# smajida/openHEVC

Measured on AMD Instinct MI355X. Metric: decoded Mpixels/s (luma), synthetic stream, higher is better.
Workload: dtype u16

## Files before the change

openhevc_amd/csrc/engine_handover.hip:

```cpp
#include <memory>

#include "engine_impl.h"

hipEvent_t sync_event_get(OhEngine *e)
{
    hipEvent_t ev = nullptr;
    if (!e->sync_events.empty()) { ev = e->sync_events.back(); e->sync_events.pop_back(); return ev; }
    return hipEventCreateWithFlags(&ev, hipEventDisableTiming) == hipSuccess ? ev : nullptr;
}
void sync_event_put(OhEngine *e, hipEvent_t ev)
{
    if (!ev) return;
    if (e->sync_events.size() < 4096) e->sync_events.push_back(ev); else (void)hipEventDestroy(ev);
}

static void *arena_new(OhEngine *e, size_t bytes)
{
    void *p = nullptr;
    if (hipMalloc(&p, bytes) != hipSuccess)
        return nullptr;
    e->arenas_alive++; e->arena_bytes_alive += bytes;
    return p;
}
static void arena_delete(OhEngine *e, void *p, size_t bytes)
{
    (void)hipFree(p);
    if (e) { e->arenas_alive--; e->arena_bytes_alive -= bytes; }
}

static int arena_take(OhEngine *e, size_t total, OhChunk *ck)
{
    int best = -1;
    for (size_t i = 0; i < e->arenas.size() && best < 0; i++)
        if (e->arenas[i].bytes >= total && e->arenas[i].bytes <= 2 * total + (1u << 20))
            best = (int)i;
    if (best >= 0 && e->arenas[best].free_ev && hipEventQuery(e->arenas[best].free_ev) != hipSuccess && e->arenas.size() < 512)
        best = -1;
    if (best >= 0) {
        ck->arena = e->arenas[best].p; ck->arena_bytes = e->arenas[best].bytes;
        if (e->arenas[best].free_ev) {
            (void)hipStreamWaitEvent(e->copy_stream, e->arenas[best].free_ev, 0);
            sync_event_put(e, e->arenas[best].free_ev);
        }
        e->arenas.erase(e->arenas.begin() + best);
        return OH_OK;
    }
    ck->arena_bytes = align_up(total, (size_t)1 << 20);
    if ((ck->arena = arena_new(e, ck->arena_bytes)) == nullptr) {
        (void)hipStreamSynchronize(e->stream);
        for (auto &a : e->arenas) { sync_event_put(e, a.free_ev); arena_delete(e, a.p, a.bytes); }
        e->arenas.clear();
        if ((ck->arena = arena_new(e, ck->arena_bytes)) == nullptr)
            FAIL(e, OH_E_NOMEM, "hipMalloc(%zu) for the work lists failed", total);
    }
    return OH_OK;
}

static void chunk_free(OhEngine *e, OhChunk *ck, bool in_flight)
{
    if (e && ck->ready)
        sync_event_put(e, ck->ready);
    if (ck->sum_host) {
        if (e && e->sum_pool.size() < 4096) e->sum_pool.push_back(ck->sum_host);
        else (void)hipHostFree(ck->sum_host);
    }
    if (ck->arena) {
        if (e && e->arenas.size() < 1024) {
            hipEvent_t fe = nullptr;
            if (in_flight && (fe = sync_event_get(e)) != nullptr && hipEventRecord(fe, e->stream) != hipSuccess) {
                sync_event_put(e, fe);
                fe = nullptr;
            }
            if (in_flight && !fe)
                (void)hipStreamSynchronize(e->stream);
            e->arenas.push_back({ ck->arena, ck->arena_bytes, fe });
        } else {
            if (in_flight && e) (void)hipStreamSynchronize(e->stream);
            arena_delete(e, ck->arena, ck->arena_bytes);
        }
    }
    delete ck;
}

void free_dev_frame(OhEngine *e, OhDevFrame *df, bool in_flight)
{
    if (!df)
        return;
    OhChunk *ck = df->chunk;
    delete df;
    if (!ck)
        return;
    ck->in_flight = ck->in_flight || in_flight;
    if (--ck->refs <= 0)
        chunk_free(e, ck, ck->in_flight);
}

static bool same_geometry(const OhPicParams &a, const OhPicParams &b)
{
    return a.width == b.width && a.height == b.height && a.bit_depth == b.bit_depth && a.chroma_format_idc == b.chroma_format_idc;
}

static int check_host_side(OhEngine *e, const OhFrame *f, const Pic *cur, HostSide *h, std::vector<uint32_t> &pu_off)
{
    const OhPicParams &p = f->p;
    h->ref_ok = 0; h->ref_used = 0; h->n_cross = 0; h->any_dense = false;
    for (int i = 0; i < OH_MAX_REFS; i++) {
        Pic *r = get_pic(e, f->ref_pics[i]);
        if (r && same_geometry(r->p, p) && r != cur)
            h->ref_ok |= 1u << i;
    }
    if ((f->n_pu && !f->pu) || (f->n_wp && !f->wp) || (f->n_tu && !f->tu) || (f->n_intra && !f->intra))
        FAIL(e, OH_E_ARG, "a non-zero item count comes with a NULL array (pu / wp / tu / intra)");
    uint64_t nl = 0, nc = 0;
    const int hs = oh_hshift(&p, 1), vs = oh_vshift(&p, 1), two = p.chroma_format_idc ? 2 : 0;
    if ((uint64_t)f->n_pu * 2048 >= (1ull << 31))
        FAIL(e, OH_E_ARG, "PU list too long");
    pu_off.resize(2 * ((size_t)f->n_pu + 1));
    uint32_t *ol = pu_off.data(), *oc = ol + f->n_pu + 1;
    h->pu_off = ol;
    for (uint32_t i = 0; i < f->n_pu; i++) {
        const OhPu &pu = f->pu[i];
        ol[i] = (uint32_t)nl; oc[i] = (uint32_t)nc;
        nl += (uint64_t)(((pu.w + 7) >> 3) * ((pu.h + 7) >> 3));
        nc += (uint64_t)(two * ((((pu.w >> hs) + 7) >> 3) * (((pu.h >> vs) + 7) >> 3)));
        for (int l = 0; l < 2; l++)
            if (pu.ref[l] < OH_MAX_REFS) h->ref_used |= (uint16_t)(1u << pu.ref[l]);
    }
    ol[f->n_pu] = (uint32_t)nl; oc[f->n_pu] = (uint32_t)nc;
    for (uint32_t i = 0; i < f->n_wp; i++)
        if (f->wp[i].log2_denom[0] > 7 || f->wp[i].log2_denom[1] > 7)
            FAIL(e, OH_E_ARG, "weights %u: log2 denominator out of range", i);
    h->tu_cnt[0] = h->tu_cnt[1] = h->tu_cnt[2] = h->tu_cnt[3] = 0;
    for (uint32_t i = 0; i < f->n_tu; i++) {
        const OhTu &t = f->tu[i];
        h->tu_cnt[(t.log2_size - 2) & 3]++;
        h->n_cross += (t.flags & OH_TUF_CROSS) != 0;
        h->any_dense = h->any_dense || !(t.flags & OH_TUF_SPARSE);
    }
    if (h->any_dense && f->n_coeff && !f->coeffs)
        FAIL(e, OH_E_ARG, "dense transform blocks but coeffs[] is NULL");
    if (h->n_cross && !f->tu_cross)
        FAIL(e, OH_E_ARG, "cross-component blocks without tu_cross[]");
    if (f->n_intra && p.constrained_intra_pred && !f->is_intra)
        FAIL(e, OH_E_ARG, "constrained_intra_pred without the is_intra map");
    if (f->n_intra) {
        if (!f->level_start || !f->n_levels || !f->ictu || !f->n_ictu || !f->sub_start || !f->n_sub ||
            f->level_start[0] != 0 || f->level_start[f->n_levels] != f->n_ictu)
            FAIL(e, OH_E_ARG, "intra wavefront tables inconsistent");
        for (uint32_t l = 0; l < f->n_levels; l++)
            if (f->level_start[l] > f->level_start[l + 1])
                FAIL(e, OH_E_ARG, "intra level table not monotonic");
    }
    if (p.deblock_enabled) {
        const OhBsInputs *bi = f->bs_in;
        if (bi && (!bi->mvf || !bi->cbf_luma || !bi->call_log2 || !bi->ctb_flags))
            FAIL(e, OH_E_ARG, "bs_in: all four maps are required");
        if (bi && (p.log2_min_pu_size < 2 || p.log2_min_tb_size < 2))
            FAIL(e, OH_E_ARG, "bs_in: min PU / TB size below 4");
        if (bi) {
            const size_t n_cells = (size_t)(p.width >> p.log2_min_tb_size) * (p.height >> p.log2_min_tb_size);
            for (size_t i = 0; i < n_cells; i++)
                if (bi->call_log2[i] && (bi->call_log2[i] < p.log2_min_tb_size || bi->call_log2[i] > p.log2_ctb_size))
                    FAIL(e, OH_E_ARG, "bs_in: call_log2[%zu] = %d is not a block size of this picture", i, bi->call_log2[i]);
        }
        if ((!bi && (!f->vertical_bs || !f->horizontal_bs || f->bs_size < oh_bs_size(&p))) || !f->qp_y_tab || !f->deblock)
            FAIL(e, OH_E_ARG, "deblock side arrays missing or too small");
    }
    if ((p.pcm_loop_filter_disable || p.transquant_bypass_enable) && !f->is_pcm)
        FAIL(e, OH_E_ARG, "is_pcm map required when pcm loop-filter disable / transquant bypass is on");
    OhPrepCounts *cnt = &h->cnt;
    cnt->n_pu = f->n_pu; cnt->n_mc_luma = (uint32_t)nl; cnt->n_mc_chroma = (uint32_t)nc; cnt->n_tu = f->n_tu;
    cnt->n_intra = f->n_intra; cnt->n_sub = f->n_intra ? f->n_sub : 0; cnt->n_ictu = f->n_intra ? f->n_ictu : 0;
    return OH_OK;
}

static void *summary_block_get(OhEngine *e)
{
    void *p = nullptr;
    if (!e->sum_pool.empty()) { p = e->sum_pool.back(); e->sum_pool.pop_back(); return p; }
    return hipHostMalloc(&p, OH_MAX_BATCH * sizeof(DevSummary), hipHostMallocDefault) == hipSuccess ? p : nullptr;
}

static void fill_header(OhEngine *e, const OhFrame *f, const Pic *cur, const HostSide &h, const HandoverLayout &L, char *copied_base, char *rest_base,
                        OhDevFrame *df, HandoverHeader *H)
{
    DevFrame &hd = H->d;
    hd.pp = f->p;
    fill_planes(&hd.cur, cur, false);
    fill_planes(&hd.out, cur, f->p.sao_enabled && f->sao);
    for (int i = 0; i < OH_MAX_REFS; i++) {
        Pic *r = get_pic(e, f->ref_pics[i]);
        df->ref_id[i] = -1; df->ref_gen[i] = 0; df->ref_half[i] = 0;
        if (h.ref_ok >> i & 1) {
            fill_planes(&hd.refs[i], r, r->final_b);
            df->ref_id[i] = f->ref_pics[i]; df->ref_gen[i] = r->gen; df->ref_half[i] = r->final_b ? 1 : 0;
        }
    }
    df->ref_used = h.ref_used;
    df->cur_gen = cur->gen;
    handover_bind_split(L, copied_base, rest_base, H);
    hd.coeffs_present = f->coeffs != nullptr;
    hd.err_word = e->kerr; hd.cur_pic_id = f->cur_pic;
    hd.n_pu = f->n_pu; hd.n_mc_luma = h.cnt.n_mc_luma; hd.n_mc_chroma = h.cnt.n_mc_chroma; hd.n_tu = f->n_tu; hd.n_intra = f->n_intra;
    hd.n_ictu = h.cnt.n_ictu; hd.n_sub = h.cnt.n_sub; hd.n_levels = f->n_intra ? f->n_levels : 0; hd.n_wp = f->n_wp; hd.n_sparse = f->sparse ? f->n_sparse : 0;
    hd.ref_ok = h.ref_ok; hd.n_coeff = f->n_coeff;
    hd.n_cross = h.n_cross;
    for (int k = 0, first = 0; k < 4; k++) { hd.tu_first[k] = (uint32_t)first; hd.tu_cnt[k] = h.tu_cnt[k]; first += (int)h.tu_cnt[k]; }
    hd.dbg = e->dbg;
}

enum { PULL_TABLE = 64 };
static_assert(HL_N_SEGS <= PULL_TABLE, "a table entry per copied segment");
static size_t pulled_stage_bytes(const HandoverLayout &L) { return L.own_bytes + PULL_TABLE * sizeof(OhPullSeg); }
static hipError_t stage_pulled(OhEngine *e, const HandoverLayout &L, char *arena, OhEngine::Stage *sg)
{
    char *sp = (char *)sg->p;
    OhPullSeg *tab = (OhPullSeg *)(sp + L.own_bytes);
    int nt = 0;
    size_t pulled = 0;
    { HostTimer t(e, OH_HT_UPLOAD_MEMCPY);
    for (int i = 0; i < L.ns; i++)
        if (L.seg[i].own && L.seg[i].bytes) {
            memcpy(sp, L.seg[i].src, L.seg[i].bytes);
            tab[nt++] = OhPullSeg{ sp, arena + L.seg[i].off, L.seg[i].bytes };
            sp += align_up(L.seg[i].bytes, 256);
        }
    for (int i = 0; i < L.ns; i++)
        if (!L.seg[i].own && L.copied(L.seg[i])) {
            tab[nt++] = OhPullSeg{ L.seg[i].src, arena + L.seg[i].off, L.seg[i].bytes };
            pulled += L.seg[i].bytes;
        }
    }
    HostTimer t_enq(e, OH_HT_UPLOAD_ENQUEUE);
    ohk_pull(tab, nt, pulled, e->copy_stream);
    return hipGetLastError();
}

static hipError_t stage_copied(OhEngine *e, const HandoverLayout *L, const size_t *copied_off, int n, char *arena, size_t bytes, OhEngine::Stage *sg)
{
    { HostTimer t(e, OH_HT_UPLOAD_MEMCPY);
    if (!e->copiers) {
        static const char *cenv = getenv("OHEVC_COPY_THREADS");
        e->copiers = new CopyPool();
        e->copiers->start(cenv ? std::max(0, std::min(atoi(cenv), 8)) : 2);
    }
    e->copy_jobs.clear();
    for (int i = 0; i < n; i++)
        handover_copy_jobs_add(L[i], (char *)sg->p + (copied_off[i] - copied_off[0]), e->copy_jobs);
    e->copiers->run(e->copy_jobs);
    }
    HostTimer t_enq(e, OH_HT_UPLOAD_ENQUEUE);
    return hipMemcpyAsync(arena + copied_off[0], sg->p, bytes, hipMemcpyHostToDevice, e->copy_stream);
}

static hipError_t enqueue_bs_derive(const OhFrame *f, const HandoverHeader &H, hipStream_t cs)
{
    const size_t bs_packed = (oh_bs_size(&f->p) + 3) / 4;
    hipError_t hrc = hipMemsetAsync((void *)H.d.vbs, 0, align_up(bs_packed, 4), cs);
    if (hrc == hipSuccess) hrc = hipMemsetAsync((void *)H.d.hbs, 0, align_up(bs_packed, 4), cs);
    if (hrc == hipSuccess)
        ohk_bs_derive(&f->p, H.mvf, H.cbf_luma, H.call_log2, H.ctb_flags, f->bs_in->loop_filter_across_tiles, (void *)H.d.vbs, (void *)H.d.hbs, cs);
    return hrc;
}

struct ChunkScratch {
    HostSide h[OH_MAX_BATCH];
    std::vector<uint32_t> pu_off[OH_MAX_BATCH];
    HandoverHeader H[OH_MAX_BATCH];
    HandoverLayout L[OH_MAX_BATCH];
    Pic *cur[OH_MAX_BATCH];
};

static int upload_chunk(OhEngine *e, const OhFrame *const *fs, int n, OhDevFrame **out)
{
    static thread_local std::unique_ptr<ChunkScratch> scratch;
    if (!scratch) scratch.reset(new ChunkScratch());
    ChunkScratch &S = *scratch;
    HostTimer t_all(e, OH_HT_UPLOAD);
    for (int i = 0; i < n; i++) {
        const OhFrame *f = fs[i];
        if (!f)
            return OH_E_ARG;
        int rc = check_params(e, &f->p);
        if (rc)
            return rc;
        S.cur[i] = get_pic(e, f->cur_pic);
        if (!S.cur[i] || !same_geometry(S.cur[i]->p, f->p))
            FAIL(e, OH_E_ARG, "cur_pic %d is not an allocated picture of this geometry", f->cur_pic);
        { HostTimer t(e, OH_HT_UPLOAD_COUNT);
        rc = check_host_side(e, f, S.cur[i], &S.h[i], S.pu_off[i]);
        }
        if (rc)
            return rc;
        memset(&S.H[i], 0, sizeof(S.H[i]));
        S.L[i] = handover_layout(f, S.h[i], &S.H[i].d);
    }
    HIPCHK(e, hipSetDevice(e->device));
    const HandoverChunk C = handover_chunk_place(S.L, n);
    OhChunk *ck = new OhChunk();
    int rc;
    { HostTimer t(e, OH_HT_UPLOAD_ARENA);
    rc = arena_take(e, C.total, ck);
    }
    if (rc) {
        delete ck;
        return rc;
    }
    if ((ck->sum_host = summary_block_get(e)) == nullptr) {
        chunk_free(e, ck, false);
        FAIL(e, OH_E_NOMEM, "hipHostMalloc(%zu) for the summaries failed", OH_MAX_BATCH * sizeof(DevSummary));
    }
    char *arena = (char *)ck->arena;
    ck->refs = n;
    for (int i = 0; i < n; i++) {
        const OhFrame *f = fs[i];
        const HostSide &h = S.h[i];
        OhDevFrame *df = new OhDevFrame();
        df->chunk = ck;
        fill_header(e, f, S.cur[i], h, S.L[i], arena + C.copied_off[i], arena + C.rest_off[i], df, &S.H[i]);
        df->sum_host = (DevSummary *)ck->sum_host + i;
        S.H[i].d.summary_host = df->sum_host;
        df->sum_dev = S.H[i].d.summary;
        df->cnt = h.cnt;
        df->d = (DevFrame *)(arena + C.copied_off[i]);
        df->p = f->p;
        for (int k = 0; k < 4; k++) df->tu_cnt[k] = h.tu_cnt[k];
        df->n_cross = h.n_cross;
        df->has_sao = f->p.sao_enabled && f->sao;
        df->cur_pic = f->cur_pic;
        df->owner = e;
        out[i] = df;
    }

    hipStream_t cs = e->copy_stream;
    auto pulled = [&](int i) { return (fs[i]->flags & OH_FRAME_PINNED) != 0 && !S.L[i].packs; };
    for (int g0 = 0, g1; g0 < n; g0 = g1) {
        const bool pull = pulled(g0);
        for (g1 = g0 + 1; !pull && g1 < n && g1 - g0 < OH_STAGE_GROUP && !pulled(g1); g1++)
            ;
        const size_t bytes = C.copied_off[g1] - C.copied_off[g0];
        OhEngine::Stage *sg;
        { HostTimer t(e, OH_HT_UPLOAD_STAGE_WAIT);
        sg = stage_acquire(e, pull ? pulled_stage_bytes(S.L[g0]) : bytes);
        }
        if (!sg)
            FAIL(e, OH_E_NOMEM, "hipHostMalloc(%zu) failed", bytes);
        hipError_t hrc = pull ? stage_pulled(e, S.L[g0], arena + C.copied_off[g0], sg)
                              : stage_copied(e, &S.L[g0], &C.copied_off[g0], g1 - g0, arena, bytes, sg);
        HostTimer t_enq(e, OH_HT_UPLOAD_ENQUEUE);
        if (hrc == hipSuccess && stage_in_use(e, sg, cs) != OH_OK)
            hrc = hipGetLastError();
        for (int i = g0; i < g1; i++) {
            e->up_bytes += S.L[i].copy_bytes;
            if (hrc == hipSuccess && S.H[i].mvf)
                hrc = enqueue_bs_derive(fs[i], S.H[i], cs);
        }
        if (hrc != hipSuccess)
            FAIL(e, OH_E_HIP, "work-list upload failed: %s", hipGetErrorString(hrc));
    }

    HostTimer t_enq(e, OH_HT_UPLOAD_ENQUEUE);
    OhBatch B;
    memset(&B, 0, sizeof(B));
    OhPrepCounts mx;
    memset(&mx, 0, sizeof(mx));
    uint32_t max_cross = 0, max_runs = 0;
    for (int i = 0; i < n; i++) {
        const OhDevFrame *df = out[i];
        B.f[i] = df->d;
        mx.n_pu = std::max(mx.n_pu, df->cnt.n_pu); mx.n_tu = std::max(mx.n_tu, df->cnt.n_tu);
        mx.n_intra = std::max(mx.n_intra, df->cnt.n_intra); mx.n_sub = std::max(mx.n_sub, df->cnt.n_sub);
        mx.n_ictu = std::max(mx.n_ictu, df->cnt.n_ictu);
        max_runs = std::max(max_runs, ((df->cnt.n_mc_luma + 63) >> 6) + ((df->cnt.n_mc_chroma + 63) >> 6));
        max_cross = std::max(max_cross, df->n_cross);
    }
    ohk_prepare(&B, n, &mx, max_runs, max_cross, cs);
    HIPCHK(e, hipGetLastError());
    if ((ck->ready = sync_event_get(e)) == nullptr)
        FAIL(e, OH_E_NOMEM, "no event for the work lists");
    HIPCHK(e, hipEventRecord(ck->ready, cs));
    return OH_OK;
}

extern "C" int oh_frames_upload(OhEngine *e, const OhFrame *const *fs, int n, OhDevFrame **out)
{
    if (!e || n < 0 || (n && (!fs || !out)))
        return OH_E_ARG;
    for (int i = 0; i < n; i++) out[i] = nullptr;
    int rc = OH_OK;
    for (int c0 = 0; c0 < n && rc == OH_OK; c0 += OH_MAX_BATCH)
        rc = upload_chunk(e, fs + c0, n - c0 < OH_MAX_BATCH ? n - c0 : OH_MAX_BATCH, out + c0);
    if (rc != OH_OK) {
        bool any = false;
        for (int i = 0; i < n; i++) any = any || out[i];
        if (any) (void)hipStreamSynchronize(e->copy_stream);
        for (int i = 0; i < n; i++) { free_dev_frame(e, out[i]); out[i] = nullptr; }
    }
    return rc;
}

extern "C" int oh_frame_upload(OhEngine *e, const OhFrame *f, OhDevFrame **out)
{
    if (!e || !f || !out)
        return OH_E_ARG;
    return oh_frames_upload(e, &f, 1, out);
}
```

openhevc_amd/csrc/engine_impl.h:

```cpp
#ifndef OHEVC_ENGINE_IMPL_H
#define OHEVC_ENGINE_IMPL_H

#include <hip/hip_runtime.h>
#include <stdio.h>
#include <stdlib.h>
#include <string.h>
#include <algorithm>
#include <chrono>
#include <string>
#include <condition_variable>
#include <mutex>
#include <thread>
#include <vector>

#include "../../include/ohevc_hip.h"
#include "handover_layout.h"
#include "kernels.h"

#define OH_INTERNAL __attribute__((visibility("hidden")))

struct Pic {
    bool        used = false;
    OhPicParams p{};
    void       *base = nullptr;
    bool        owned = true;
    void       *a[3] = {}, *b[3] = {};
    int32_t     stride[3] = {}, w[3] = {}, h[3] = {};
    bool        final_b = false;
    uint32_t    gen = 0;
    uint64_t    done_seq = 0;
};

struct EventSet { hipEvent_t ev[OH_N_PASSES + 1]; int n_frames = 1; };

struct OhChunk {
    void      *arena = nullptr;
    size_t     arena_bytes = 0;
    hipEvent_t ready = nullptr;
    bool       waited = false;
    void      *sum_host = nullptr;
    int        refs = 0;
    bool       in_flight = false;
};

struct OhDevFrame {
    OhChunk   *chunk = nullptr;
    DevFrame  *d = nullptr;
    OhPicParams p{};
    uint32_t   tu_cnt[4] = { 0, 0, 0, 0 };
    uint32_t   n_cross = 0;
    bool       has_sao = false;
    int        cur_pic = -1;
    uint32_t   cur_gen = 0;
    int        ref_id[OH_MAX_REFS];
    uint32_t   ref_gen[OH_MAX_REFS];
    uint8_t    ref_half[OH_MAX_REFS];
    uint16_t   ref_used = 0;
    void      *sum_host = nullptr;
    bool       summary_read = false;
    void      *sum_dev = nullptr;
    OhPrepCounts cnt{};
    uint32_t   prep_err = 0;
    uint32_t   intra_area64 = 0, max_passes = 0;
    uint32_t   max_items = 0, max_sub = 0, max_res = 0;
    bool       res_scattered = false;
    uint64_t   sum_items = 0, sum_sub = 0;
    const struct OhEngine *owner = nullptr;
};

struct CopyPool {
    std::vector<std::thread> th;
    std::mutex mu;
    std::condition_variable cv, done_cv;
    const std::vector<CopyJob> *jobs = nullptr;
    int pending = 0;
    uint64_t gen = 0;
    bool stop = false;
    static void run_share(const std::vector<CopyJob> &jobs, int share, int shares)
    {
        for (size_t i = (size_t)share; i < jobs.size(); i += (size_t)shares) {
            const CopyJob &j = jobs[i];
            if (j.pack) pack_bs((uint8_t *)j.dst, (const uint8_t *)j.src, j.n);
            else memcpy(j.dst, j.src, j.n);
        }
    }
    void worker(int k)
    {
        uint64_t seen = 0;
        for (;;) {
            const std::vector<CopyJob> *my;
            {
                std::unique_lock<std::mutex> lk(mu);
                cv.wait(lk, [&] { return stop || gen != seen; });
                if (stop) return;
                seen = gen;
                my = jobs;
            }
            run_share(*my, k + 1, (int)th.size() + 1);
            {
                std::lock_guard<std::mutex> lk(mu);
                if (--pending == 0) done_cv.notify_one();
            }
        }
    }
    void start(int n) { for (int k = 0; k < n; k++) th.emplace_back(&CopyPool::worker, this, k); }
    void run(const std::vector<CopyJob> &j)
    {
        if (th.empty()) { run_share(j, 0, 1); return; }
        {
            std::lock_guard<std::mutex> lk(mu);
            jobs = &j; pending = (int)th.size(); gen++;
        }
        cv.notify_all();
        run_share(j, 0, (int)th.size() + 1);
        std::unique_lock<std::mutex> lk(mu);
        done_cv.wait(lk, [&] { return pending == 0; });
    }
    ~CopyPool()
    {
        { std::lock_guard<std::mutex> lk(mu); stop = true; }
        cv.notify_all();
        for (auto &t : th) t.join();
    }
};

struct OhEngine {
    int         device = 0;
    int         n_cu = 256;
    hipStream_t stream = nullptr;
    bool        own_stream = true;
    std::vector<Pic> pics;
    std::string err;
    int         profile = 0;
    std::vector<EventSet> ev_pool, ev_pending;
    std::vector<hipEvent_t> lev_pool, lev_pending;
    double      intra_launch_ms = 0;
    uint64_t    intra_launches = 0;
    double      pass_ms[OH_N_PASSES] = {};
    uint64_t    executes = 0;
    std::vector<OhDevFrame *> deferred;
    uint32_t    pic_gen = 0;
    struct Stage { void *p; size_t bytes; hipEvent_t done; bool busy; };
    std::vector<Stage> stages;
    hipStream_t copy_stream = nullptr;
    struct Arena { void *p; size_t bytes; hipEvent_t free_ev; };
    std::vector<Arena> arenas;
    uint64_t    arenas_alive = 0, arena_bytes_alive = 0;
    std::vector<hipEvent_t> sync_events;
    std::vector<void *> sum_pool;
    double      host_ms[OH_N_HOST_TIMES] = {};
    uint64_t    host_calls[OH_N_HOST_TIMES] = {};
    uint64_t    up_bytes = 0;
    uint64_t   *dbg = nullptr;
    enum { BATCH_RING = 64 };
    hipEvent_t  batch_ev[BATCH_RING] = {};
    uint64_t    batch_seq = 0;
    hipStream_t dl_stream = nullptr;
    enum { TICKET_RING = 128, TICKET_WORDS = 2 * OH_MAX_BATCH * 32 };
    uint32_t   *tickets = nullptr;
    uint64_t    ticket_seq = 0;
    CopyPool   *copiers = nullptr;
    std::mutex  dl_mu, dl_copy_mu;
    std::vector<Stage *> dl_stages;
    CopyPool   *dl_copiers = nullptr;
    std::vector<CopyJob> dl_jobs;
    double      dl_wait_ms = 0, dl_copy_ms = 0;
    uint64_t    dl_count = 0;
    std::vector<CopyJob> copy_jobs;
    uint32_t   *kerr = nullptr;
    struct Scratch { void *p = nullptr; size_t bytes = 0; };
    Scratch     hash_dev;
    Scratch     resize_dev;
    struct TableCache {
        OhColour last;
        bool     cached = false, on_dev = false;
        std::vector<int32_t> tab;
        int32_t  misc[OH_COL_NMISC];
        Scratch  dev;
    };
    TableCache  colour_tabs;
    TableCache  light_tabs;
    Scratch     light_res;
    Scratch     compare_res;
    Scratch     compose_dev;
    uint32_t    spin_limit = 1u << 22;
};

#define HIPCHK(e, call)                                                                           \
    do {                                                                                          \
        hipError_t rc_ = (call);                                                                  \
        if (rc_ != hipSuccess) {                                                                  \
            char buf_[512];                                                                       \
            snprintf(buf_, sizeof(buf_), "%s failed: %s (%s:%d)", #call, hipGetErrorString(rc_), __FILE__, __LINE__); \
            (e)->err = buf_;                                                                      \
            return OH_E_HIP;                                                                      \
        }                                                                                         \
    } while (0)

#define FAIL(e, code, ...)                                                                        \
    do {                                                                                          \
        char buf_[512];                                                                           \
        snprintf(buf_, sizeof(buf_), __VA_ARGS__);                                                \
        (e)->err = buf_;                                                                          \
        return (code);                                                                            \
    } while (0)

struct HostTimer {
    OhEngine *e; int slot; std::chrono::steady_clock::time_point t0;
    HostTimer(OhEngine *e_, int slot_);
    ~HostTimer();
};
enum : size_t { OH_STAGE_POOL_BYTES = (size_t)48 * ((size_t)4 << 20) };
#ifndef OH_STAGE_GROUP
#define OH_STAGE_GROUP 32
#endif

static inline void *const *final_planes(const Pic *p) { return p->final_b ? p->b : p->a; }
static inline int sample_bytes(int bit_depth) { return bit_depth > 8 ? 2 : 1; }
static inline void fill_planes(DevPlanes *dp, const Pic *p, bool use_b)
{
    for (int c = 0; c < 3; c++) {
        dp->p[c] = use_b ? p->b[c] : p->a[c];
        dp->stride[c] = p->stride[c];
        dp->w[c] = p->w[c];
        dp->h[c] = p->h[c];
    }
}

OH_INTERNAL int kernel_error(OhEngine *e);
OH_INTERNAL int check_params(OhEngine *e, const OhPicParams *p);
OH_INTERNAL Pic *get_pic(OhEngine *e, int id);
OH_INTERNAL int check_pics(OhEngine *e, const int *pic_ids, int n, const char *who);
OH_INTERNAL bool stage_create(OhEngine::Stage *c, size_t bytes);
OH_INTERNAL OhEngine::Stage *stage_acquire(OhEngine *e, size_t bytes);
OH_INTERNAL OhEngine::Stage *stage_list(OhEngine *e, const void *list, size_t bytes);
OH_INTERNAL int stage_in_use(OhEngine *e, OhEngine::Stage *sg, hipStream_t st);
OH_INTERNAL hipEvent_t sync_event_get(OhEngine *e);
OH_INTERNAL void sync_event_put(OhEngine *e, hipEvent_t ev);
OH_INTERNAL void free_dev_frame(OhEngine *e, OhDevFrame *df, bool in_flight = false);

#endif
```

openhevc_amd/csrc/handover_layout.h:

```cpp
#ifndef OHEVC_HANDOVER_LAYOUT_H
#define OHEVC_HANDOVER_LAYOUT_H

#include <stddef.h>
#include <string.h>
#include <algorithm>
#include <vector>

#include "dev_frame.h"

static inline size_t align_up(size_t v, size_t a) { return (v + a - 1) / a * a; }

static inline void pack_bs(uint8_t *dst, const uint8_t *src, size_t n)
{
    size_t i = 0;
    for (; i + 4 <= n; i += 4) {
        uint32_t x;
        memcpy(&x, src + i, 4);
        dst[i >> 2] = (uint8_t)(((x & 0x03030303u) * 0x01041040u) >> 24);
    }
    if (i < n) {
        uint32_t v = 0;
        for (size_t k = i; k < n; k++) v |= (uint32_t)(src[k] & 3) << ((k & 3) * 2);
        dst[i >> 2] = (uint8_t)v;
    }
}

struct HostSide {
    OhPrepCounts cnt;
    uint32_t tu_cnt[4], n_cross;
    bool     any_dense;
    uint16_t ref_used;
    uint32_t ref_ok;
    const uint32_t *pu_off;
};

struct HandoverHeader { DevFrame d; char *mvf, *cbf_luma, *call_log2, *ctb_flags; };
#define HL_FIELD(m) offsetof(HandoverHeader, m)
enum : size_t { HL_NO_FIELD = ~(size_t)0 };

struct HandoverSeg {
    const void *src;
    size_t bytes, field;
    bool   null_field;
    bool   own;
    size_t pack_n;
    size_t off;
};
enum { HL_OPT = 1, HL_OWN = 2 };
static inline HandoverSeg hl_in(bool have, const void *src, size_t bytes, size_t field, int how = 0, size_t pack_n = 0)
{
    return HandoverSeg{ have ? src : nullptr, have ? bytes : 0, field, (how & HL_OPT) && !have, (how & HL_OWN) != 0, pack_n, 0 };
}
static inline HandoverSeg hl_dev(size_t bytes, size_t field) { return HandoverSeg{ nullptr, bytes, field, false, false, 0, 0 }; }

enum { HL_N_SEGS = 43 };
struct HandoverLayout {
    HandoverSeg seg[HL_N_SEGS];
    int    ns;
    size_t copy_bytes;
    size_t zero_off, zero_bytes;
    size_t res_off, stale_off, stale_bytes, total;
    size_t own_bytes;
    bool   packs;
    bool copied(const HandoverSeg &s) const { return s.bytes && s.src && s.off + s.bytes <= copy_bytes; }
};

template <size_t N> static inline void hl_place(HandoverLayout *L, const HandoverSeg (&segs)[N])
{
    for (const HandoverSeg &s : segs) {
        HandoverSeg &d = L->seg[L->ns++];
        d = s;
        d.off = L->total;
        L->total += align_up(s.bytes ? s.bytes : 1, 256);
        if (s.own) L->own_bytes += align_up(s.bytes, 256);
    }
}

static inline HandoverLayout handover_layout(const OhFrame *f, const HostSide &h, const DevFrame *hdr)
{
    const OhPicParams &p = f->p;
    const OhPrepCounts &cnt = h.cnt;
    const size_t n_ctb = (size_t)oh_ctb_width(&p) * oh_ctb_height(&p);
    const size_t n_pcm = (size_t)oh_min_pu_width(&p) * oh_min_pu_height(&p);
    const size_t n_mtb = (size_t)(p.width >> p.log2_min_tb_size) * (p.height >> p.log2_min_tb_size);
    const bool has_sao = p.sao_enabled && f->sao;
    const bool has_db = p.deblock_enabled != 0;
    const uint32_t n_levels = f->n_intra ? f->n_levels : 0;
    const bool cip = p.constrained_intra_pred && f->is_intra;
    static const OhBsInputs no_maps{};
    const bool bsi = has_db && f->bs_in;
    const OhBsInputs &bm = bsi ? *f->bs_in : no_maps;
    const size_t bs_bytes = bsi ? oh_bs_size(&p) : f->bs_size;
    const size_t bs_packed = (bs_bytes + 3) / 4;
    const bool packs = has_db && !bsi && !(f->flags & OH_FRAME_BS_PACKED);
    const bool need_pcm = f->is_pcm && (p.pcm_loop_filter_disable || p.transquant_bypass_enable);
    const bool has_pend = has_sao && f->sao_pending && oh_sao_stale_config(&p);

    const HandoverSeg copied[] = {
        hl_in(true, hdr, sizeof(DevFrame), HL_NO_FIELD, HL_OWN),
        hl_in(true, f->pu, (size_t)f->n_pu * sizeof(OhPu), HL_FIELD(d.pu)),
        hl_in(true, h.pu_off, 2 * ((size_t)f->n_pu + 1) * sizeof(uint32_t), HL_FIELD(d.pu_off), HL_OWN),
        hl_in(true, f->wp, (size_t)f->n_wp * sizeof(OhWeights), HL_FIELD(d.wp)),
        hl_in(true, f->tu, (size_t)f->n_tu * sizeof(OhTu), HL_FIELD(d.tu_raw)),
        hl_in(f->tu_sparse, f->tu_sparse, (size_t)f->n_tu * sizeof(uint32_t), HL_FIELD(d.tu_sparse), HL_OPT),
        hl_in(f->tu_cross, f->tu_cross, (size_t)f->n_tu * sizeof(uint32_t), HL_FIELD(d.tu_cross), HL_OPT),
        hl_in(f->sparse, f->sparse, (size_t)f->n_sparse * sizeof(uint32_t), HL_FIELD(d.sparse), HL_OPT),
        hl_in(f->scaling, f->scaling, sizeof(OhScalingList), HL_FIELD(d.scaling), HL_OPT),
        hl_in(true, f->intra, (size_t)f->n_intra * sizeof(OhIntra), HL_FIELD(d.intra_raw)),
        hl_in(cnt.n_ictu, f->ictu, (size_t)cnt.n_ictu * sizeof(OhIntraCtu), HL_FIELD(d.ictu_raw)),
        hl_in(n_levels, f->level_start, ((size_t)n_levels + 1) * sizeof(uint32_t), HL_FIELD(d.lvl_start)),
        hl_in(cnt.n_sub, f->sub_start, ((size_t)cnt.n_sub + 1) * sizeof(uint32_t), HL_FIELD(d.sub_start)),
        hl_in(cip, f->is_intra, n_pcm, HL_FIELD(d.is_intra), HL_OPT),
        hl_in(has_db, bsi ? nullptr : f->vertical_bs, bs_packed, HL_FIELD(d.vbs), 0, packs ? bs_bytes : 0),
        hl_in(has_db, bsi ? nullptr : f->horizontal_bs, bs_packed, HL_FIELD(d.hbs), 0, packs ? bs_bytes : 0),
        hl_in(bsi, bm.mvf, n_pcm * sizeof(OhMvField), HL_FIELD(mvf), HL_OPT),
        hl_in(bsi, bm.cbf_luma, n_mtb, HL_FIELD(cbf_luma), HL_OPT),
        hl_in(bsi, bm.call_log2, n_mtb, HL_FIELD(call_log2), HL_OPT),
        hl_in(bsi, bm.ctb_flags, n_ctb, HL_FIELD(ctb_flags), HL_OPT),
        hl_in(has_db, f->qp_y_tab, oh_qp_tab_size(&p), HL_FIELD(d.qp)),
        hl_in(need_pcm, f->is_pcm, n_pcm, HL_FIELD(d.is_pcm), HL_OPT),
        hl_in(has_db, f->deblock, n_ctb * sizeof(OhDeblockCtb), HL_FIELD(d.db)),
        hl_in(has_sao, f->sao, n_ctb * sizeof(OhSaoCtb), HL_FIELD(d.sao), HL_OPT),
        hl_in(has_pend, f->sao_pending, n_ctb, HL_FIELD(d.sao_pending), HL_OPT),
        hl_in(true, f->coeffs, (size_t)f->n_coeff * sizeof(int16_t), HL_FIELD(d.coeffs)),
    };
    const HandoverSeg cleared[] = {
        hl_dev(16 * sizeof(uint32_t), HL_FIELD(d.tu_cursor)),
        hl_dev(sizeof(DevSummary), HL_FIELD(d.summary)),
        hl_dev(cnt.n_intra ? n_ctb * sizeof(uint32_t) : 0, HL_FIELD(d.ctu_seen)),
        hl_dev(f->n_tu, HL_FIELD(d.tu_keep)),
    };
    const HandoverSeg device[] = {
        hl_dev((size_t)cnt.n_mc_luma * sizeof(DevMcJob), HL_FIELD(d.mc_luma)),
        hl_dev((size_t)cnt.n_mc_chroma * sizeof(DevMcJob), HL_FIELD(d.mc_chroma)),
        hl_dev((size_t)cnt.n_ictu * sizeof(uint32_t), HL_FIELD(d.ctu_aux)),
        hl_dev((size_t)f->n_tu * sizeof(DevTu), HL_FIELD(d.tu)),
        hl_dev((size_t)h.n_cross * sizeof(DevCross), HL_FIELD(d.cross)),
        hl_dev((size_t)f->n_intra * sizeof(DevIntra), HL_FIELD(d.intra)),
        hl_dev((size_t)cnt.n_ictu * sizeof(DevIntraCtu), HL_FIELD(d.ictu)),
        hl_dev((size_t)cnt.n_sub * sizeof(uint32_t), HL_FIELD(d.sub_small)),
        hl_dev((size_t)f->n_intra * sizeof(uint32_t), HL_FIELD(d.intra_perm)),
        hl_dev((size_t)cnt.n_ictu * 4 * sizeof(uint32_t), HL_FIELD(d.ctu_wait)),
        hl_dev((size_t)cnt.n_ictu * sizeof(uint32_t), HL_FIELD(d.ctu_done)),
        hl_dev((size_t)cnt.n_ictu * sizeof(uint32_t), HL_FIELD(d.ctu_lvl)),
        hl_dev((size_t)cnt.n_ictu * sizeof(uint32_t), HL_FIELD(d.ctu_order)),
    };
    static_assert(sizeof(copied) + sizeof(cleared) + sizeof(device) == HL_N_SEGS * sizeof(HandoverSeg), "HandoverLayout::seg[] holds exactly the segments stated here");

    HandoverLayout L;
    L.ns = 0; L.total = 0; L.own_bytes = 0; L.packs = packs;
    hl_place(&L, copied);
    L.copy_bytes = h.any_dense || !f->n_tu ? L.total : L.seg[L.ns - 1].off;
    L.zero_off = L.total;
    hl_place(&L, cleared);
    L.zero_bytes = L.total - L.zero_off;
    hl_place(&L, device);
    L.res_off = L.total;
    L.total += align_up((size_t)(f->n_coeff ? f->n_coeff : 1) * sizeof(int16_t), 256);
    L.stale_off = L.total;
    L.stale_bytes = has_db && has_sao && oh_sao_stale_config(&p) ? oh_sao_stale_index(&p, 3, 0, 0) * sizeof(uint16_t) : 0;
    if (L.stale_bytes)
        L.total += align_up(L.stale_bytes, 256);
    return L;
}

static inline char *hl_at(const HandoverLayout &L, char *copied_base, char *rest_base, size_t off)
{
    return off < L.copy_bytes ? copied_base + off : rest_base + (off - L.copy_bytes);
}

static inline void handover_bind_split(const HandoverLayout &L, char *copied_base, char *rest_base, HandoverHeader *H)
{
    for (int i = 0; i < L.ns; i++)
        if (L.seg[i].field != HL_NO_FIELD) {
            char *at = L.seg[i].null_field ? nullptr : hl_at(L, copied_base, rest_base, L.seg[i].off);
            memcpy((char *)H + L.seg[i].field, &at, sizeof(at));
        }
    H->d.sub_small_w = (uint32_t *)H->d.sub_small;
    H->d.res = (int16_t *)hl_at(L, copied_base, rest_base, L.res_off);
    H->d.sao_stale = L.stale_bytes ? (uint16_t *)hl_at(L, copied_base, rest_base, L.stale_off) : nullptr;
    H->d.zero_ptr = (uint32_t *)hl_at(L, copied_base, rest_base, L.zero_off); H->d.zero_words = (uint32_t)(L.zero_bytes / 4);
}

static inline void handover_bind(const HandoverLayout &L, char *base, HandoverHeader *H)
{
    handover_bind_split(L, base, base + L.copy_bytes, H);
}

struct HandoverChunk {
    int    n;
    size_t copied_off[OH_MAX_BATCH + 1];
    size_t rest_off[OH_MAX_BATCH];
    size_t copy_bytes, total;
};
static inline HandoverChunk handover_chunk_place(const HandoverLayout *L, int n)
{
    HandoverChunk C;
    memset(&C, 0, sizeof(C));
    C.n = n;
    size_t at = 0;
    for (int i = 0; i < n; i++) { C.copied_off[i] = at; at += align_up(L[i].copy_bytes, 256); }
    C.copied_off[n] = C.copy_bytes = at;
    for (int i = 0; i < n; i++) { C.rest_off[i] = at; at += align_up(L[i].total - L[i].copy_bytes, 256); }
    C.total = at;
    return C;
}

struct CopyJob { char *dst; const char *src; size_t n; bool pack; };
static inline void handover_copy_jobs_add(const HandoverLayout &L, char *stage, std::vector<CopyJob> &jobs)
{
    const size_t piece = 128 * 1024;
    for (int i = 0; i < L.ns; i++) {
        const HandoverSeg &s = L.seg[i];
        if (!L.copied(s))
            continue;
        const size_t n = s.pack_n ? s.pack_n : s.bytes, step = s.pack_n ? 4 * piece : piece;
        for (size_t o = 0; o < n; o += step)
            jobs.push_back({ stage + s.off + (s.pack_n ? o / 4 : o), (const char *)s.src + o, std::min(step, n - o), s.pack_n != 0 });
    }
}
static inline void handover_copy_jobs(const HandoverLayout &L, char *stage, std::vector<CopyJob> &jobs)
{
    jobs.clear();
    handover_copy_jobs_add(L, stage, jobs);
}

#endif
```

Measured before the change: 78970.

## Parallelize per-frame host validation across copy pool and vectorize bs packing

Moves the per-frame host-side checks and PU offset counting into a header function and runs it for all frames of a chunk in parallel on the copy thread pool, which is rewritten as a generic work-stealing pool with an atomic index. The pack_bs routine gains a 32-byte vector path that packs eight words per iteration. The TU dense-flag scan becomes a branchless AND reduction. This targets host CPU time in the upload path, but adds thread wake and synchronisation overhead per chunk and slightly changes error-ordering semantics.

```diff
diff --git a/openhevc_amd/csrc/engine_handover.hip b/openhevc_amd/csrc/engine_handover.hip
--- a/openhevc_amd/csrc/engine_handover.hip
+++ b/openhevc_amd/csrc/engine_handover.hip
@@ -100,78 +100,25 @@
     return a.width == b.width && a.height == b.height && a.bit_depth == b.bit_depth && a.chroma_format_idc == b.chroma_format_idc;
 }
 
-static int check_host_side(OhEngine *e, const OhFrame *f, const Pic *cur, HostSide *h, std::vector<uint32_t> &pu_off)
-{
-    const OhPicParams &p = f->p;
-    h->ref_ok = 0; h->ref_used = 0; h->n_cross = 0; h->any_dense = false;
+static CopyPool *copiers_get(OhEngine *e)
+{
+    if (!e->copiers) {
+        static const char *cenv = getenv("OHEVC_COPY_THREADS");
+        e->copiers = new CopyPool();
+        e->copiers->start(cenv ? std::max(0, std::min(atoi(cenv), 8)) : 2);
+    }
+    return e->copiers;
+}
+
+static uint32_t usable_refs(OhEngine *e, const OhFrame *f, const Pic *cur)
+{
+    uint32_t ok = 0;
     for (int i = 0; i < OH_MAX_REFS; i++) {
         Pic *r = get_pic(e, f->ref_pics[i]);
-        if (r && same_geometry(r->p, p) && r != cur)
-            h->ref_ok |= 1u << i;
-    }
-    if ((f->n_pu && !f->pu) || (f->n_wp && !f->wp) || (f->n_tu && !f->tu) || (f->n_intra && !f->intra))
-        FAIL(e, OH_E_ARG, "a non-zero item count comes with a NULL array (pu / wp / tu / intra)");
-    uint64_t nl = 0, nc = 0;
-    const int hs = oh_hshift(&p, 1), vs = oh_vshift(&p, 1), two = p.chroma_format_idc ? 2 : 0;
-    if ((uint64_t)f->n_pu * 2048 >= (1ull << 31))
-        FAIL(e, OH_E_ARG, "PU list too long");
-    pu_off.resize(2 * ((size_t)f->n_pu + 1));
-    uint32_t *ol = pu_off.data(), *oc = ol + f->n_pu + 1;
-    h->pu_off = ol;
-    for (uint32_t i = 0; i < f->n_pu; i++) {
-        const OhPu &pu = f->pu[i];
-        ol[i] = (uint32_t)nl; oc[i] = (uint32_t)nc;
-        nl += (uint64_t)(((pu.w + 7) >> 3) * ((pu.h + 7) >> 3));
-        nc += (uint64_t)(two * ((((pu.w >> hs) + 7) >> 3) * (((pu.h >> vs) + 7) >> 3)));
-        for (int l = 0; l < 2; l++)
-            if (pu.ref[l] < OH_MAX_REFS) h->ref_used |= (uint16_t)(1u << pu.ref[l]);
-    }
-    ol[f->n_pu] = (uint32_t)nl; oc[f->n_pu] = (uint32_t)nc;
-    for (uint32_t i = 0; i < f->n_wp; i++)
-        if (f->wp[i].log2_denom[0] > 7 || f->wp[i].log2_denom[1] > 7)
-            FAIL(e, OH_E_ARG, "weights %u: log2 denominator out of range", i);
-    h->tu_cnt[0] = h->tu_cnt[1] = h->tu_cnt[2] = h->tu_cnt[3] = 0;
-    for (uint32_t i = 0; i < f->n_tu; i++) {
-        const OhTu &t = f->tu[i];
-        h->tu_cnt[(t.log2_size - 2) & 3]++;
-        h->n_cross += (t.flags & OH_TUF_CROSS) != 0;
-        h->any_dense = h->any_dense || !(t.flags & OH_TUF_SPARSE);
-    }
-    if (h->any_dense && f->n_coeff && !f->coeffs)
-        FAIL(e, OH_E_ARG, "dense transform blocks but coeffs[] is NULL");
-    if (h->n_cross && !f->tu_cross)
-        FAIL(e, OH_E_ARG, "cross-component blocks without tu_cross[]");
-    if (f->n_intra && p.constrained_intra_pred && !f->is_intra)
-        FAIL(e, OH_E_ARG, "constrained_intra_pred without the is_intra map");
-    if (f->n_intra) {
-        if (!f->level_start || !f->n_levels || !f->ictu || !f->n_ictu || !f->sub_start || !f->n_sub ||
-            f->level_start[0] != 0 || f->level_start[f->n_levels] != f->n_ictu)
-            FAIL(e, OH_E_ARG, "intra wavefront tables inconsistent");
-        for (uint32_t l = 0; l < f->n_levels; l++)
-            if (f->level_start[l] > f->level_start[l + 1])
-                FAIL(e, OH_E_ARG, "intra level table not monotonic");
-    }
-    if (p.deblock_enabled) {
-        const OhBsInputs *bi = f->bs_in;
-        if (bi && (!bi->mvf || !bi->cbf_luma || !bi->call_log2 || !bi->ctb_flags))
-            FAIL(e, OH_E_ARG, "bs_in: all four maps are required");
-        if (bi && (p.log2_min_pu_size < 2 || p.log2_min_tb_size < 2))
-            FAIL(e, OH_E_ARG, "bs_in: min PU / TB size below 4");
-        if (bi) {
-            const size_t n_cells = (size_t)(p.width >> p.log2_min_tb_size) * (p.height >> p.log2_min_tb_size);
-            for (size_t i = 0; i < n_cells; i++)
-                if (bi->call_log2[i] && (bi->call_log2[i] < p.log2_min_tb_size || bi->call_log2[i] > p.log2_ctb_size))
-                    FAIL(e, OH_E_ARG, "bs_in: call_log2[%zu] = %d is not a block size of this picture", i, bi->call_log2[i]);
-        }
-        if ((!bi && (!f->vertical_bs || !f->horizontal_bs || f->bs_size < oh_bs_size(&p))) || !f->qp_y_tab || !f->deblock)
-            FAIL(e, OH_E_ARG, "deblock side arrays missing or too small");
-    }
-    if ((p.pcm_loop_filter_disable || p.transquant_bypass_enable) && !f->is_pcm)
-        FAIL(e, OH_E_ARG, "is_pcm map required when pcm loop-filter disable / transquant bypass is on");
-    OhPrepCounts *cnt = &h->cnt;
-    cnt->n_pu = f->n_pu; cnt->n_mc_luma = (uint32_t)nl; cnt->n_mc_chroma = (uint32_t)nc; cnt->n_tu = f->n_tu;
-    cnt->n_intra = f->n_intra; cnt->n_sub = f->n_intra ? f->n_sub : 0; cnt->n_ictu = f->n_intra ? f->n_ictu : 0;
-    return OH_OK;
+        if (r && same_geometry(r->p, f->p) && r != cur)
+            ok |= 1u << i;
+    }
+    return ok;
 }
 
 static void *summary_block_get(OhEngine *e)
@@ -239,15 +186,10 @@
 static hipError_t stage_copied(OhEngine *e, const HandoverLayout *L, const size_t *copied_off, int n, char *arena, size_t bytes, OhEngine::Stage *sg)
 {
     { HostTimer t(e, OH_HT_UPLOAD_MEMCPY);
-    if (!e->copiers) {
-        static const char *cenv = getenv("OHEVC_COPY_THREADS");
-        e->copiers = new CopyPool();
-        e->copiers->start(cenv ? std::max(0, std::min(atoi(cenv), 8)) : 2);
-    }
     e->copy_jobs.clear();
     for (int i = 0; i < n; i++)
         handover_copy_jobs_add(L[i], (char *)sg->p + (copied_off[i] - copied_off[0]), e->copy_jobs);
-    e->copiers->run(e->copy_jobs);
+    copiers_get(e)->run(e->copy_jobs);
     }
     HostTimer t_enq(e, OH_HT_UPLOAD_ENQUEUE);
     return hipMemcpyAsync(arena + copied_off[0], sg->p, bytes, hipMemcpyHostToDevice, e->copy_stream);
@@ -269,6 +211,8 @@
     HandoverHeader H[OH_MAX_BATCH];
     HandoverLayout L[OH_MAX_BATCH];
     Pic *cur[OH_MAX_BATCH];
+    uint32_t ref_ok[OH_MAX_BATCH];
+    HandoverCheck chk[OH_MAX_BATCH];
 };
 
 static int upload_chunk(OhEngine *e, const OhFrame *const *fs, int n, OhDevFrame **out)
@@ -277,23 +221,35 @@
     if (!scratch) scratch.reset(new ChunkScratch());
     ChunkScratch &S = *scratch;
     HostTimer t_all(e, OH_HT_UPLOAD);
-    for (int i = 0; i < n; i++) {
+    CopyPool *pool = copiers_get(e);
+    int n_ok = 0, rc_engine = OH_OK;
+    auto engine_side = [&](int i) -> int {
         const OhFrame *f = fs[i];
         if (!f)
             return OH_E_ARG;
-        int rc = check_params(e, &f->p);
-        if (rc)
+        if (const int rc = check_params(e, &f->p))
             return rc;
         S.cur[i] = get_pic(e, f->cur_pic);
         if (!S.cur[i] || !same_geometry(S.cur[i]->p, f->p))
             FAIL(e, OH_E_ARG, "cur_pic %d is not an allocated picture of this geometry", f->cur_pic);
-        { HostTimer t(e, OH_HT_UPLOAD_COUNT);
-        rc = check_host_side(e, f, S.cur[i], &S.h[i], S.pu_off[i]);
-        }
-        if (rc)
-            return rc;
+        S.ref_ok[i] = usable_refs(e, f, S.cur[i]);
+        return OH_OK;
+    };
+    while (n_ok < n && (rc_engine = engine_side(n_ok)) == OH_OK)
+        n_ok++;
+    int bad;
+    { HostTimer t(e, OH_HT_UPLOAD_COUNT);
+    bad = handover_check_chunk(pool, fs, S.ref_ok, n_ok, S.h, S.pu_off, S.chk);
+    }
+    if (bad >= 0) {
+        e->err = S.chk[bad].msg;
+        return S.chk[bad].rc;
+    }
+    if (rc_engine != OH_OK)
+        return rc_engine;
+    for (int i = 0; i < n; i++) {
         memset(&S.H[i], 0, sizeof(S.H[i]));
-        S.L[i] = handover_layout(f, S.h[i], &S.H[i].d);
+        S.L[i] = handover_layout(fs[i], S.h[i], &S.H[i].d);
     }
     HIPCHK(e, hipSetDevice(e->device));
     const HandoverChunk C = handover_chunk_place(S.L, n);
diff --git a/openhevc_amd/csrc/engine_impl.h b/openhevc_amd/csrc/engine_impl.h
--- a/openhevc_amd/csrc/engine_impl.h
+++ b/openhevc_amd/csrc/engine_impl.h
@@ -15,6 +15,7 @@
 
 #include "../../include/ohevc_hip.h"
 #include "handover_layout.h"
+#include "handover_host.h"
 #include "kernels.h"
 
 #define OH_INTERNAL __attribute__((visibility("hidden")))
@@ -66,62 +67,6 @@
     bool       res_scattered = false;
     uint64_t   sum_items = 0, sum_sub = 0;
     const struct OhEngine *owner = nullptr;
-};
-
-struct CopyPool {
-    std::vector<std::thread> th;
-    std::mutex mu;
-    std::condition_variable cv, done_cv;
-    const std::vector<CopyJob> *jobs = nullptr;
-    int pending = 0;
-    uint64_t gen = 0;
-    bool stop = false;
-    static void run_share(const std::vector<CopyJob> &jobs, int share, int shares)
-    {
-        for (size_t i = (size_t)share; i < jobs.size(); i += (size_t)shares) {
-            const CopyJob &j = jobs[i];
-            if (j.pack) pack_bs((uint8_t *)j.dst, (const uint8_t *)j.src, j.n);
-            else memcpy(j.dst, j.src, j.n);
-        }
-    }
-    void worker(int k)
-    {
-        uint64_t seen = 0;
-        for (;;) {
-            const std::vector<CopyJob> *my;
-            {
-                std::unique_lock<std::mutex> lk(mu);
-                cv.wait(lk, [&] { return stop || gen != seen; });
-                if (stop) return;
-                seen = gen;
-                my = jobs;
-            }
-            run_share(*my, k + 1, (int)th.size() + 1);
-            {
-                std::lock_guard<std::mutex> lk(mu);
-                if (--pending == 0) done_cv.notify_one();
-            }
-        }
-    }
-    void start(int n) { for (int k = 0; k < n; k++) th.emplace_back(&CopyPool::worker, this, k); }
-    void run(const std::vector<CopyJob> &j)
-    {
-        if (th.empty()) { run_share(j, 0, 1); return; }
-        {
-            std::lock_guard<std::mutex> lk(mu);
-            jobs = &j; pending = (int)th.size(); gen++;
-        }
-        cv.notify_all();
-        run_share(j, 0, (int)th.size() + 1);
-        std::unique_lock<std::mutex> lk(mu);
-        done_cv.wait(lk, [&] { return pending == 0; });
-    }
-    ~CopyPool()
-    {
-        { std::lock_guard<std::mutex> lk(mu); stop = true; }
-        cv.notify_all();
-        for (auto &t : th) t.join();
-    }
 };
 
 struct OhEngine {
diff --git a/openhevc_amd/csrc/handover_host.h b/openhevc_amd/csrc/handover_host.h
--- /dev/null
+++ b/openhevc_amd/csrc/handover_host.h
@@ -0,0 +1,192 @@
+#ifndef OHEVC_HANDOVER_HOST_H
+#define OHEVC_HANDOVER_HOST_H
+
+#include <stdarg.h>
+#include <stdio.h>
+#include <atomic>
+#include <condition_variable>
+#include <mutex>
+#include <thread>
+#include <type_traits>
+#include <vector>
+
+#include "../../include/ohevc_hip.h"
+#include "handover_layout.h"
+
+struct HandoverCheck { int rc; char msg[200]; };
+
+static inline int hc_fail(HandoverCheck *r, int code, const char *fmt, ...) __attribute__((format(printf, 3, 4)));
+static inline int hc_fail(HandoverCheck *r, int code, const char *fmt, ...)
+{
+    va_list ap;
+    va_start(ap, fmt);
+    vsnprintf(r->msg, sizeof(r->msg), fmt, ap);
+    va_end(ap);
+    return r->rc = code;
+}
+
+static inline int handover_check_list(const OhFrame *f, uint32_t ref_ok, HostSide *h, std::vector<uint32_t> &pu_off, HandoverCheck *r)
+{
+    const OhPicParams &p = f->p;
+    r->rc = OH_OK; r->msg[0] = 0;
+    h->ref_ok = ref_ok; h->ref_used = 0; h->n_cross = 0; h->any_dense = false;
+    if ((f->n_pu && !f->pu) || (f->n_wp && !f->wp) || (f->n_tu && !f->tu) || (f->n_intra && !f->intra))
+        return hc_fail(r, OH_E_ARG, "a non-zero item count comes with a NULL array (pu / wp / tu / intra)");
+    uint64_t nl = 0, nc = 0;
+    const int hs = oh_hshift(&p, 1), vs = oh_vshift(&p, 1), two = p.chroma_format_idc ? 2 : 0;
+    if ((uint64_t)f->n_pu * 2048 >= (1ull << 31))
+        return hc_fail(r, OH_E_ARG, "PU list too long");
+    pu_off.resize(2 * ((size_t)f->n_pu + 1));
+    uint32_t *ol = pu_off.data(), *oc = ol + f->n_pu + 1;
+    h->pu_off = ol;
+    uint32_t ref_used = 0;
+    for (uint32_t i = 0; i < f->n_pu; i++) {
+        const OhPu &pu = f->pu[i];
+        ol[i] = (uint32_t)nl; oc[i] = (uint32_t)nc;
+        nl += (uint64_t)(((pu.w + 7) >> 3) * ((pu.h + 7) >> 3));
+        nc += (uint64_t)(two * ((((pu.w >> hs) + 7) >> 3) * (((pu.h >> vs) + 7) >> 3)));
+        for (int l = 0; l < 2; l++)
+            if (pu.ref[l] < OH_MAX_REFS) ref_used |= 1u << pu.ref[l];
+    }
+    h->ref_used = (uint16_t)ref_used;
+    ol[f->n_pu] = (uint32_t)nl; oc[f->n_pu] = (uint32_t)nc;
+    for (uint32_t i = 0; i < f->n_wp; i++)
+        if (f->wp[i].log2_denom[0] > 7 || f->wp[i].log2_denom[1] > 7)
+            return hc_fail(r, OH_E_ARG, "weights %u: log2 denominator out of range", i);
+    uint32_t tu_cnt[4] = { 0, 0, 0, 0 }, n_cross = 0, all_flags = OH_TUF_SPARSE;
+    for (uint32_t i = 0; i < f->n_tu; i++) {
+        const OhTu &t = f->tu[i];
+        tu_cnt[(t.log2_size - 2) & 3]++;
+        n_cross += (t.flags & OH_TUF_CROSS) != 0;
+        all_flags &= t.flags;
+    }
+    for (int k = 0; k < 4; k++) h->tu_cnt[k] = tu_cnt[k];
+    h->n_cross = n_cross;
+    h->any_dense = f->n_tu && !(all_flags & OH_TUF_SPARSE);
+    if (h->any_dense && f->n_coeff && !f->coeffs)
+        return hc_fail(r, OH_E_ARG, "dense transform blocks but coeffs[] is NULL");
+    if (h->n_cross && !f->tu_cross)
+        return hc_fail(r, OH_E_ARG, "cross-component blocks without tu_cross[]");
+    if (f->n_intra && p.constrained_intra_pred && !f->is_intra)
+        return hc_fail(r, OH_E_ARG, "constrained_intra_pred without the is_intra map");
+    if (f->n_intra) {
+        if (!f->level_start || !f->n_levels || !f->ictu || !f->n_ictu || !f->sub_start || !f->n_sub ||
+            f->level_start[0] != 0 || f->level_start[f->n_levels] != f->n_ictu)
+            return hc_fail(r, OH_E_ARG, "intra wavefront tables inconsistent");
+        for (uint32_t l = 0; l < f->n_levels; l++)
+            if (f->level_start[l] > f->level_start[l + 1])
+                return hc_fail(r, OH_E_ARG, "intra level table not monotonic");
+    }
+    if (p.deblock_enabled) {
+        const OhBsInputs *bi = f->bs_in;
+        if (bi && (!bi->mvf || !bi->cbf_luma || !bi->call_log2 || !bi->ctb_flags))
+            return hc_fail(r, OH_E_ARG, "bs_in: all four maps are required");
+        if (bi && (p.log2_min_pu_size < 2 || p.log2_min_tb_size < 2))
+            return hc_fail(r, OH_E_ARG, "bs_in: min PU / TB size below 4");
+        if (bi) {
+            const size_t n_cells = (size_t)(p.width >> p.log2_min_tb_size) * (p.height >> p.log2_min_tb_size);
+            for (size_t i = 0; i < n_cells; i++)
+                if (bi->call_log2[i] && (bi->call_log2[i] < p.log2_min_tb_size || bi->call_log2[i] > p.log2_ctb_size))
+                    return hc_fail(r, OH_E_ARG, "bs_in: call_log2[%zu] = %d is not a block size of this picture", i, bi->call_log2[i]);
+        }
+        if ((!bi && (!f->vertical_bs || !f->horizontal_bs || f->bs_size < oh_bs_size(&p))) || !f->qp_y_tab || !f->deblock)
+            return hc_fail(r, OH_E_ARG, "deblock side arrays missing or too small");
+    }
+    if ((p.pcm_loop_filter_disable || p.transquant_bypass_enable) && !f->is_pcm)
+        return hc_fail(r, OH_E_ARG, "is_pcm map required when pcm loop-filter disable / transquant bypass is on");
+    OhPrepCounts *cnt = &h->cnt;
+    cnt->n_pu = f->n_pu; cnt->n_mc_luma = (uint32_t)nl; cnt->n_mc_chroma = (uint32_t)nc; cnt->n_tu = f->n_tu;
+    cnt->n_intra = f->n_intra; cnt->n_sub = f->n_intra ? f->n_sub : 0; cnt->n_ictu = f->n_intra ? f->n_ictu : 0;
+    return OH_OK;
+}
+
+struct CopyPool {
+    std::vector<std::thread> th;
+    std::mutex mu;
+    std::condition_variable cv, done_cv;
+    void (*call)(void *ctx, size_t i) = nullptr;
+    void *ctx = nullptr;
+    size_t n_items = 0;
+    std::atomic<size_t> next{ 0 };
+    uint64_t gen = 0;
+    bool open = false;
+    int joined = 0, finished = 0;
+    bool stop = false;
+
+    void worker()
+    {
+        uint64_t seen = 0;
+        std::unique_lock<std::mutex> lk(mu);
+        for (;;) {
+            cv.wait(lk, [&] { return stop || (open && gen != seen); });
+            if (stop) return;
+            seen = gen;
+            joined++;
+            void (*const c)(void *, size_t) = call;
+            void *const x = ctx;
+            const size_t n = n_items;
+            lk.unlock();
+            for (size_t i; (i = next.fetch_add(1, std::memory_order_relaxed)) < n; )
+                c(x, i);
+            lk.lock();
+            if (++finished == joined && !open) done_cv.notify_one();
+        }
+    }
+    void start(int n) { for (int k = 0; k < n; k++) th.emplace_back(&CopyPool::worker, this); }
+    int helpers() const { return (int)th.size(); }
+
+    template <class Fn> void run(size_t n, Fn &&fn, int max_helpers = 1 << 30)
+    {
+        const size_t k = std::min({ th.size(), (size_t)std::max(max_helpers, 0), n ? n - 1 : 0 });
+        if (!k) {
+            for (size_t i = 0; i < n; i++) fn(i);
+            return;
+        }
+        {
+            std::lock_guard<std::mutex> lk(mu);
+            ctx = (void *)&fn;
+            call = [](void *x, size_t i) { (*(typename std::remove_reference<Fn>::type *)x)(i); };
+            n_items = n;
+            next.store(0, std::memory_order_relaxed);
+            joined = finished = 0;
+            open = true; gen++;
+        }
+        if (k == th.size()) cv.notify_all();
+        else for (size_t i = 0; i < k; i++) cv.notify_one();
+        for (size_t i; (i = next.fetch_add(1, std::memory_order_relaxed)) < n; )
+            fn(i);
+        std::unique_lock<std::mutex> lk(mu);
+        open = false;
+        done_cv.wait(lk, [&] { return finished == joined; });
+    }
+    static void copy_one(const CopyJob &j)
+    {
+        if (j.pack) pack_bs((uint8_t *)j.dst, (const uint8_t *)j.src, j.n);
+        else memcpy(j.dst, j.src, j.n);
+    }
+    void run(const std::vector<CopyJob> &jobs)
+    {
+        const CopyJob *j = jobs.data();
+        run(jobs.size(), [j](size_t i) { copy_one(j[i]); });
+    }
+    ~CopyPool()
+    {
+        { std::lock_guard<std::mutex> lk(mu); stop = true; }
+        cv.notify_all();
+        for (auto &t : th) t.join();
+    }
+};
+
+static inline int handover_check_chunk(CopyPool *pool, const OhFrame *const *fs, const uint32_t *ref_ok, int n, HostSide *h,
+                                       std::vector<uint32_t> *pu_off, HandoverCheck *res)
+{
+    auto one = [=](size_t i) { (void)handover_check_list(fs[i], ref_ok[i], &h[i], pu_off[i], &res[i]); };
+    if (pool) pool->run((size_t)n, one);
+    else for (int i = 0; i < n; i++) one((size_t)i);
+    for (int i = 0; i < n; i++)
+        if (res[i].rc != OH_OK)
+            return i;
+    return -1;
+}
+
+#endif
diff --git a/openhevc_amd/csrc/handover_layout.h b/openhevc_amd/csrc/handover_layout.h
--- a/openhevc_amd/csrc/handover_layout.h
+++ b/openhevc_amd/csrc/handover_layout.h
@@ -12,7 +12,18 @@
 
 static inline void pack_bs(uint8_t *dst, const uint8_t *src, size_t n)
 {
+    typedef uint32_t pb_u32x8 __attribute__((vector_size(32)));
+    typedef uint8_t pb_u8x8 __attribute__((vector_size(8)));
     size_t i = 0;
+    for (; i + 32 <= n; i += 32) {
+        pb_u32x8 x;
+        memcpy(&x, src + i, 32);
+        x &= 0x03030303u;
+        x |= x >> 6;
+        x = (x | (x >> 12)) & 0xffu;
+        const pb_u8x8 y = __builtin_convertvector(x, pb_u8x8);
+        memcpy(dst + (i >> 2), &y, 8);
+    }
     for (; i + 4 <= n; i += 4) {
         uint32_t x;
         memcpy(&x, src + i, 4);
```

Result: faster. 85710 (median of 6 runs) (+8.5%).
